# Gjerman/Orange3-Spark

Hardware: AMD Instinct MI355X
Metric: samples/sec LogisticRegression.fit on 1Bx256 synthetic at 1/2/4/8 MI355X (higher is better)
Workload: dtype bf16; 1 GPU; global_batch=1000000000, seq_len=256, features=256, parallelism=dp1, resident_rows=497795896, lineage_rows=502204104, device=cuda:0

## Files before the change

### orange3_spark_amd/ops/csrc/glm.hip

```cpp
#include <type_traits>

#include "common.h"

using namespace o3s;

namespace {

enum { LOSS_LOGISTIC = 0, LOSS_HINGE = 1, LOSS_SQUARED = 2 };

constexpr int kBlock = 256;
constexpr int kWavesPerBlock = kBlock / kWave;

__host__ __device__ __forceinline__ uint32_t umad24(uint32_t a, uint32_t c, uint32_t add) {
#if defined(__HIP_DEVICE_COMPILE__)
  return __umul24(a, c) + add;
#else
  return (a & 0xFFFFFFu) * c + add;
#endif
}
__host__ __device__ __forceinline__ uint32_t mix24(uint32_t h) {
  h ^= h >> 16;
  h = umad24(h, 0xED5AD4u, h);
  h ^= h >> 15;
  return umad24(h, 0x2C1B3Cu, h);
// ... 268 lines not shown
  wtshift *= kSynthShift;
  float acc_r = 0.f, acc_loss = 0.f, acc_w = 0.f;

  const int64_t ntiles = (n + RT - 1) / RT;
  const int64_t gw = (int64_t)blockIdx.x * kWavesPerBlock + wid;
  const int64_t nw = (int64_t)gridDim.x * kWavesPerBlock;
  for (int64_t t = gw; t < ntiles; t += nw) {
    const int64_t base = t * RT;
    short8 xv[UNROLL][CPL];
    float xf[UNROLL][CPL][8];
#pragma unroll
    for (int u = 0; u < UNROLL; ++u) {
      const int64_t row = base + u * G + g;
      const bool ok = row < n;
      const int64_t rowc = ok ? row : n - 1;
      const uint32_t rk = SRC == 1 ? feat_key(seed, row0 + row) : 0u;
#pragma unroll
      for (int k = 0; k < CPL; ++k) {
        const int ch = c + k * LPR;
        if (SRC == 0) {
          const bool okc = ok && ch < nch;
          const int chc = ch < nch ? ch : nch - 1;
          short8 v = __builtin_nontemporal_load(reinterpret_cast<const short8*>(X + rowc * ld + 8 * chc));
          xv[u][k] = okc ? v : short8{0, 0, 0, 0, 0, 0, 0, 0};
        } else {
          const uint32_t h0 = synth_word(rk, 2 * ch), h1 = synth_word(rk, 2 * ch + 1);
#pragma unroll
          for (int j = 0; j < 4; ++j) {
            xf[u][k][j] = synth_byte(h0, j);
            xf[u][k][4 + j] = synth_byte(h1, j);
          }
        }
      }
    }
    float yy[NF], ww[NF];
#pragma unroll
    for (int j = 0; j < NF; ++j) {
      const int64_t row = base + (ubase + j) * G + g;
      const bool ok = row < n;
      const int64_t rowc = ok ? row : n - 1;
      if (SRC == 0) {
        const float yv = y[rowc];
        const float wv = sw ? sw[rowc] : 1.f;
        yy[j] = ok ? yv : 0.f;
        ww[j] = ok ? wv : 0.f;
      } else {
        ww[j] = ok ? 1.f : 0.f;
      }
    }
    float dot[UNROLL], dtrue[UNROLL];
#pragma unroll
    for (int u = 0; u < UNROLL; ++u) {
      float d = SRC == 1 ? wshift : 0.f, dt = wtshift;
#pragma unroll
      for (int k = 0; k < CPL; ++k) {
        float x[8];
        if (SRC == 0) {
          unpack8(xv[u][k], x);
        } else {
#pragma unroll
          for (int j = 0; j < 8; ++j) x[j] = xf[u][k][j];
        }
#pragma unroll
        for (int j = 0; j < 8; ++j) {
          d = fmaf(x[j], w[k][j], d);
          if (SRC == 1) dt = fmaf(x[j], wt[k][j], dt);
        }
      }
      dot[u] = d;
      dtrue[u] = dt;
    }
    RR::run(dot, c);
    if (SRC == 1) {
      RR::run(dtrue, c);
#pragma unroll
      for (int j = 0; j < NF; ++j) {
        const int64_t row = base + (ubase + j) * G + g;
        yy[j] = synth_label(row_key(seed, row0 + row), dtrue[j] + btrue);
      }
    }
    float res[NF];
#pragma unroll
    for (int j = 0; j < NF; ++j) {
      float r, l;
      loss_terms<LOSS>(dot[j] + intercept, yy[j], ww[j], r, l);
      res[j] = r;
      if (rep) { acc_r += r; acc_loss += l; acc_w += ww[j]; }
    }
#pragma unroll
    for (int u = 0; u < UNROLL; ++u)
#pragma unroll
      for (int k = 0; k < CPL; ++k) {
        if (SRC == 0) asm volatile("" : "+v"(xv[u][k]));
        else {
#pragma unroll
          for (int j = 0; j < 8; ++j) asm volatile("" : "+v"(xf[u][k][j]));
        }
      }
#pragma unroll
    for (int u = 0; u < UNROLL; ++u) {
      float r = __shfl(res[u % NF], g * LPR + RR::owner(u), kWave);
      if (SRC == 1) { rs += r; r *= kSynthScale; }
#pragma unroll
      for (int k = 0; k < CPL; ++k) {
        float x[8];
        if (SRC == 0) {
          unpack8(xv[u][k], x);
        } else {
#pragma unroll
          for (int j = 0; j < 8; ++j) x[j] = xf[u][k][j];
        }
#pragma unroll
        for (int j = 0; j < 8; ++j) acc[k][j] = fmaf(r, x[j], acc[k][j]);
      }
    }
  }

  if (SRC == 1) {
#pragma unroll
    for (int k = 0; k < CPL; ++k)
#pragma unroll
      for (int j = 0; j < 8; ++j) acc[k][j] = fmaf(rs, kSynthShift, acc[k][j]);
  }
  grad_epilogue<LPR, CPL>(acc, acc_r, acc_loss, acc_w, partial, pstride, 0, lane, wid, c);
}


template <int CTRL>
__device__ __forceinline__ float dpp_f(float v) {
  return __builtin_bit_cast(float, __builtin_amdgcn_update_dpp(0, __builtin_bit_cast(int, v), CTRL, 0xF, 0xF,
                                                               false));
}
constexpr int kDppXor1 = 0xB1, kDppXor2 = 0x4E, kDppHalfMirror = 0x141;
__device__ __forceinline__ void row_reduce_8x2(float (&v)[2], int c) {
  v[0] += dpp_f<kDppXor1>(v[0]);
  v[1] += dpp_f<kDppXor1>(v[1]);
  v[0] += dpp_f<kDppXor2>(v[0]);
  v[1] += dpp_f<kDppXor2>(v[1]);
  const bool up = (c & 4) != 0;
  const float keep = up ? v[1] : v[0], send = up ? v[0] : v[1];
  v[0] = keep + dpp_f<kDppHalfMirror>(send);
}

struct RowSampler {
  uint32_t key, thr;
  int64_t grow0;
  __device__ __forceinline__ bool on() const { return thr < (1u << 24); }
  __device__ __forceinline__ bool keep(int64_t row) const { return (row_key(key, grow0 + row) >> 8) < thr; }
};
__host__ __device__ __forceinline__ uint32_t sample_key(uint32_t seed, uint32_t iter) {
  return fmix32(seed ^ fmix32(iter * 0x9E3779B1u + 0x7F4A7C15u));
}

constexpr int kStgTileBytes = 8 * 1024, kStgLabelBytes = kWave * 4;
constexpr int kStgWaveBytes = kStgTileBytes + 2 * kStgLabelBytes;
constexpr int kStgLd = 256;
constexpr unsigned kAuxNt = 2;
struct TileStage {
  static constexpr int LPR = 8, CPL = 4, UNROLL = 2, G = kWave / LPR, kTileOps = 1 + UNROLL * CPL;
  unsigned char* slot;
  uint32_t sbase;
  const unsigned char* xs;
  const float* yrs;
  const float* yls;
  int64_t tstep;
  uint32_t r_ahead, l_ahead;
  bool lab_younger;

  __device__ static __forceinline__ uint32_t fresh(int v) {
    asm volatile("" : "+v"(v));
    return (uint32_t)v;
  }
  __device__ static __forceinline__ uint32_t label_off(uint32_t g, uint32_t c) { return ((c >> 2) * G + g) * 4; }

  __device__ __forceinline__ void issue_tile(int g, int c) {
    const uint32_t gg = fresh(g), cc = fresh(c);
    __builtin_amdgcn_global_load_lds(reinterpret_cast<const unsigned char*>(yrs) + label_off(gg, cc),
                                     slot + kStgTileBytes, 4, 0, 0);
    const uint32_t xoff = gg * (kStgLd * 2) + cc * 16;
#pragma unroll
    for (int u = 0; u < UNROLL; ++u)
#pragma unroll
      for (int k = 0; k < CPL; ++k)
        __builtin_amdgcn_global_load_lds(xs + (u * G * kStgLd * 2 + k * LPR * 16) + xoff, slot + (u * CPL + k) * 1024,
                                         16, 0, kAuxNt);
    xs += tstep * (kStgLd * 2);
    yrs += tstep;
    --r_ahead;
    lab_younger = false;
  }
  __device__ __forceinline__ void issue_label(int g, int c) {
    __builtin_amdgcn_global_load_lds(reinterpret_cast<const unsigned char*>(yls) + label_off(fresh(g), fresh(c)),
                                     slot + kStgTileBytes + kStgLabelBytes, 4, 0, 0);
    yls += tstep;
    --l_ahead;
    lab_younger = true;
  }
  __device__ __forceinline__ void take_tile(int g, int c, short8 (&xv)[UNROLL][CPL], float& yv) {
    if (lab_younger) asm volatile("s_waitcnt vmcnt(1)" ::: "memory");
    else asm volatile("s_waitcnt vmcnt(0)" ::: "memory");
    const uint32_t lane = fresh(g) * LPR + fresh(c);
    asm volatile(
        "ds_read_b128 %0, %9\n\t"
        "ds_read_b128 %1, %9 offset:1024\n\t"
        "ds_read_b128 %2, %9 offset:2048\n\t"
        "ds_read_b128 %3, %9 offset:3072\n\t"
        "ds_read_b128 %4, %9 offset:4096\n\t"
        "ds_read_b128 %5, %9 offset:5120\n\t"
        "ds_read_b128 %6, %9 offset:6144\n\t"
        "ds_read_b128 %7, %9 offset:7168\n\t"
        "ds_read_b32 %8, %10 offset:8192\n\t"
        "s_waitcnt lgkmcnt(0)"
        : "=&v"(xv[0][0]), "=&v"(xv[0][1]), "=&v"(xv[0][2]), "=&v"(xv[0][3]), "=&v"(xv[1][0]), "=&v"(xv[1][1]),
          "=&v"(xv[1][2]), "=&v"(xv[1][3]), "=&v"(yv)
        : "v"(sbase + lane * 16), "v"(sbase + lane * 4)
        : "memory");
    if (r_ahead > 0) issue_tile(g, c);
    __builtin_amdgcn_sched_barrier(0);
  }
  __device__ __forceinline__ void take_label(int g, int c, float& yv) {
    if (lab_younger) asm volatile("s_waitcnt vmcnt(0)" ::: "memory");
    else asm volatile("s_waitcnt vmcnt(%0)" ::"n"(kTileOps) : "memory");
    const uint32_t a4 = sbase + (fresh(g) * LPR + fresh(c)) * 4;
    asm volatile("ds_read_b32 %0, %1 offset:8448\n\ts_waitcnt lgkmcnt(0)" : "=v"(yv) : "v"(a4) : "memory");
    lab_younger = false;
    if (l_ahead > 0) issue_label(g, c);
  }
};
static_assert(kStgTileBytes == 8192 && kStgLabelBytes == 256, "the asm offsets in TileStage");

template <class SRC, int LPR, int CPL, int UNROLL, int LOSS, bool SMP, bool FULL = false, bool STAGED = false>
__device__ __forceinline__ void grad_tile(
    int64_t base, int64_t n, const typename SRC::elem* __restrict__ X, int64_t ld, int nch,
    const float* __restrict__ y, const float* __restrict__ sw, uint32_t seed, int64_t row0, const float (&w)[CPL][8],
    float wshift, float intercept, int g, int c, const RowSampler smp, float (&acc)[CPL][8], float& rs, float& acc_r,
    float& acc_loss, float& acc_w, TileStage* stg = nullptr) {
  constexpr int G = kWave / LPR;
  using RR = RowReduce<LPR, UNROLL>;
  constexpr int NF = RR::NF;
  static_assert(!STAGED || (FULL && NF == 1 && LPR == TileStage::LPR && CPL == TileStage::CPL && UNROLL == TileStage::UNROLL),
                "the staged slot holds one (8, 4, 2) tile");
  const int ubase = RR::base(c);
  const bool rep = RR::representative(c);
  typename SRC::chunk xv[UNROLL][CPL];
#pragma unroll
  for (int u = 0; u < UNROLL; ++u) {
    const int64_t row = base + u * G + g;
    const bool ok = row < n;
    const int64_t rowc = ok ? row : n - 1;
    const uint32_t fk = SRC::kLineage ? feat_key(seed, row0 + row) : 0u;
#pragma unroll
    for (int k = 0; k < CPL; ++k) {
      const int ch = c + k * LPR;
      if constexpr (SRC::kLineage) {
        SRC::decode(synth_word(fk, 2 * ch), synth_word(fk, 2 * ch + 1), xv[u][k]);
      } else if constexpr (STAGED) {
      } else if constexpr (FULL) {
        SRC::load(X, ld, row, ch, xv[u][k]);
      } else {
        const int chc = ch < nch ? ch : nch - 1;
        SRC::load(X, ld, rowc, chc, xv[u][k]);
        SRC::mask(xv[u][k], ok && ch < nch);
      }
    }
  }
  float yy[NF], ww[NF];
#pragma unroll
  for (int j = 0; j < NF; ++j) {
    const int64_t row = base + (ubase + j) * G + g;
    const bool ok = row < n;
    const int64_t rowc = ok ? row : n - 1;
    if constexpr (STAGED) {
      if constexpr (!SRC::kLineage) stg->take_tile(g, c, xv, yy[j]);
      ww[j] = 1.f;
    } else if constexpr (FULL) {
      yy[j] = y[row];
      ww[j] = sw ? sw[row] : 1.f;
    } else {
      const float yv = y[rowc];
      const float wv = sw ? sw[rowc] : 1.f;
      yy[j] = ok ? yv : 0.f;
      ww[j] = ok ? wv : 0.f;
    }
    if constexpr (SMP && !STAGED) {
      if (!smp.keep(row)) ww[j] = 0.f;
    }
  }
  float dot[UNROLL];
#pragma unroll
  for (int u = 0; u < UNROLL; ++u) {
    float2_ d2 = {0.f, 0.f};
#pragma unroll
    for (int k = 0; k < CPL; ++k) {
      float x[8];
      SRC::unpack(xv[u][k], x);
#pragma unroll
      for (int j = 0; j < 8; j += 2) {
        const float2_ xx = {x[j], x[j + 1]}, ww2 = {w[k][j], w[k][j + 1]};
        d2 = __builtin_elementwise_fma(xx, ww2, d2);
      }
    }
    dot[u] = SRC::dot(d2.x + d2.y, wshift);
  }
  constexpr bool kDpp = LPR == 8 && UNROLL == 2;
  if constexpr (kDpp) row_reduce_8x2(dot, c);
  else RR::run(dot, c);
  if constexpr (STAGED && SRC::kLineage) stg->take_label(g, c, yy[0]);
  if constexpr (STAGED && SMP) {
    if (!smp.keep(base + (int64_t)TileStage::fresh(ubase * G + g))) ww[0] = 0.f;
  }
  float res[NF];
#pragma unroll
  for (int j = 0; j < NF; ++j) {
    float r, l;
    loss_terms<LOSS>(dot[j] + intercept, yy[j], ww[j], r, l);
    res[j] = r;
    if (rep) { acc_r += r; acc_loss += l; acc_w += ww[j]; }
  }
#pragma unroll
  for (int u = 0; u < UNROLL; ++u)
#pragma unroll
    for (int k = 0; k < CPL; ++k) SRC::pin(xv[u][k]);
  float other = 0.f;
  if constexpr (kDpp) other = dpp_f<kDppHalfMirror>(res[0]);
#pragma unroll
  for (int u = 0; u < UNROLL; ++u) {
    float r;
    if constexpr (kDpp) r = ((c & 4) != 0) == (u == 0) ? other : res[0];
    else r = __shfl(res[u % NF], g * LPR + RR::owner(u), kWave);
    r = SRC::resid(r, rs);
#pragma unroll
    for (int k = 0; k < CPL; ++k) {
      float x[8];
      SRC::unpack(xv[u][k], x);
#pragma unroll
      for (int j = 0; j < 8; ++j) acc[k][j] = fmaf(r, x[j], acc[k][j]);
    }
  }
}

template <int LPR, int CPL, int UNROLL, int LOSS, int MW, bool SMP, bool FULL = false>
__global__ __launch_bounds__(kBlock, MW) void glm_grad_mixed_kernel(
    const uint16_t* __restrict__ X, int64_t ld, int64_t n_res, const float* __restrict__ y,
    const float* __restrict__ sw, const float* __restrict__ y_lin, const float* __restrict__ sw_lin,
    const float* __restrict__ coef, const float* __restrict__ bptr, uint32_t seed, int64_t row0, int64_t n_lin,
    float* __restrict__ partial, int pstride, int64_t res_row0, const int64_t* __restrict__ t_dev, uint32_t sseed,
    uint32_t sthr, int pacc) {
  constexpr int G = kWave / LPR;
  constexpr int RT = G * UNROLL;
  const int lane = threadIdx.x & (kWave - 1);
  const int wid = threadIdx.x / kWave;
  const int g = lane / LPR, c = lane % LPR;
  const int nch = (int)(ld / 8);
  const float intercept = *bptr;
  const uint32_t skey = SMP ? sample_key(sseed, (uint32_t)((t_dev ? t_dev[0] : 0) + 1)) : 0u;
  const RowSampler smp_res{skey, sthr, res_row0}, smp_lin{skey, sthr, row0};

  float w[CPL][8], acc[CPL][8];
  float wshift = 0.f;
#pragma unroll
  for (int k = 0; k < CPL; ++k)
#pragma unroll
    for (int j = 0; j < 8; ++j) {
      const int col = 8 * (c + k * LPR) + j;
      w[k][j] = col < ld ? coef[col] : 0.f;
      wshift += w[k][j];
      acc[k][j] = 0.f;
    }
  wshift *= kSynthShift;
  float rs = 0.f;
  float acc_r = 0.f, acc_loss = 0.f, acc_w = 0.f;

  const int64_t Tr = (n_res + RT - 1) / RT, Tl = (n_lin + RT - 1) / RT, S = Tr + Tl;
  const int64_t gw = (int64_t)blockIdx.x * kWavesPerBlock + wid;
  const int64_t nw = (int64_t)gridDim.x * kWavesPerBlock;
  if (gw < S) {
    int64_t L = gw * Tl / S, rem = gw * Tl - L * S;
    const int64_t q0 = nw * Tl / S, r0 = nw * Tl - q0 * S;
    for (int64_t s = gw; s < S; s += nw) {
      if (rem + Tl >= S)
        grad_tile<RowsLineage, LPR, CPL, UNROLL, LOSS, SMP, FULL>(L * RT, n_lin, X, ld, nch, y_lin, sw_lin, seed, row0, w,
                                                                  wshift, intercept, g, c, smp_lin, acc, rs, acc_r, acc_loss,
                                                                  acc_w);
      else
        grad_tile<RowsBf16, LPR, CPL, UNROLL, LOSS, SMP, FULL>((s - L) * RT, n_res, X, ld, nch, y, sw, seed, row0, w, wshift,
                                                               intercept, g, c, smp_res, acc, rs, acc_r, acc_loss, acc_w);
      rem += r0;
      L += q0;
      if (rem >= S) { rem -= S; ++L; }
    }
  }
#pragma unroll
  for (int k = 0; k < CPL; ++k)
#pragma unroll
    for (int j = 0; j < 8; ++j) acc[k][j] = fmaf(rs, kSynthShift, acc[k][j]);
  grad_epilogue<LPR, CPL>(acc, acc_r, acc_loss, acc_w, partial, pstride, pacc, lane, wid, c);
}

template <int LOSS, bool SMP>
__global__ __launch_bounds__(kBlock, 3) void glm_grad_staged_kernel(
    const uint16_t* __restrict__ X, int64_t n_res, const float* __restrict__ y, const float* __restrict__ y_lin,
    const float* __restrict__ coef, const float* __restrict__ bptr, uint32_t seed, int64_t row0, int64_t n_lin,
    float* __restrict__ partial, int pstride, int64_t res_row0, const int64_t* __restrict__ t_dev, uint32_t sseed,
    uint32_t sthr, int pacc) {
  constexpr int LPR = TileStage::LPR, CPL = TileStage::CPL, UNROLL = TileStage::UNROLL, G = TileStage::G;
  constexpr int RT = G * UNROLL;
  constexpr int64_t ld = kStgLd;
  __shared__ __attribute__((aligned(16))) unsigned char slots[kWavesPerBlock * kStgWaveBytes];
  const int lane = threadIdx.x & (kWave - 1);
  const int wid = __builtin_amdgcn_readfirstlane(threadIdx.x / kWave);
  const int g = lane / LPR, c = lane % LPR;
  const float intercept = *bptr;
  const uint32_t skey = SMP ? sample_key(sseed, (uint32_t)((t_dev ? t_dev[0] : 0) + 1)) : 0u;
  const RowSampler smp_res{skey, sthr, res_row0}, smp_lin{skey, sthr, row0};

  float w[CPL][8], acc[CPL][8];
  float wshift = 0.f;
#pragma unroll
  for (int k = 0; k < CPL; ++k)
#pragma unroll
    for (int j = 0; j < 8; ++j) {
      w[k][j] = coef[8 * (c + k * LPR) + j];
      wshift += w[k][j];
      acc[k][j] = 0.f;
    }
  wshift *= kSynthShift;
  float rs = 0.f;
  float acc_r = 0.f, acc_loss = 0.f, acc_w = 0.f;

  const uint32_t Tr = (uint32_t)(n_res / RT), Tl = (uint32_t)(n_lin / RT);
  const uint32_t gw = blockIdx.x * kWavesPerBlock + wid, nw = gridDim.x * kWavesPerBlock;
  const uint32_t nr = gw < Tr ? (Tr - gw + nw - 1) / nw : 0u;
  const uint32_t nl = gw < Tl ? (Tl - gw + nw - 1) / nw : 0u;
  const uint32_t S = nr + nl;
  int64_t br = (int64_t)gw * RT, bl = br;
  using lds_byte = __attribute__((address_space(3))) unsigned char;
  TileStage st{slots + wid * kStgWaveBytes,
               (uint32_t)(uintptr_t)(lds_byte*)slots + wid * kStgWaveBytes,
               reinterpret_cast<const unsigned char*>(X + br * ld),
               y + br,
               y_lin + bl,
               (int64_t)nw * RT,
               nr,
               nl,
               false};
  static_assert(RowReduce<LPR, UNROLL>::NF == 1, "TileStage::label_off: one label per lane");
  if (nl > 0) st.issue_label(g, c);
  if (nr > 0) st.issue_tile(g, c);
  uint32_t rem = 0;
  for (uint32_t s = 0; s < S; ++s) {
    rem += nl;
    if (rem >= S) {
      rem -= S;
      grad_tile<RowsLineage, LPR, CPL, UNROLL, LOSS, SMP, true, true>(bl, n_lin, X, ld, CPL * LPR, y_lin, nullptr, seed, row0,
                                                                      w, wshift, intercept, g, c, smp_lin, acc, rs, acc_r,
                                                                      acc_loss, acc_w, &st);
      bl += st.tstep;
    } else {
      grad_tile<RowsBf16, LPR, CPL, UNROLL, LOSS, SMP, true, true>(br, n_res, X, ld, CPL * LPR, y, nullptr, seed, row0, w,
                                                                   wshift, intercept, g, c, smp_res, acc, rs, acc_r,
                                                                   acc_loss, acc_w, &st);
      br += st.tstep;
    }
  }
#pragma unroll
  for (int k = 0; k < CPL; ++k)
#pragma unroll
    for (int j = 0; j < 8; ++j) acc[k][j] = fmaf(rs, kSynthShift, acc[k][j]);
  grad_epilogue<LPR, CPL>(acc, acc_r, acc_loss, acc_w, partial, pstride, pacc, lane, wid, c);
}

template <class SRC, int LPR, int CPL, int U, bool UNW, bool FULL = false>
__device__ __forceinline__ void stats_tile(int64_t base, int64_t n, const typename SRC::elem* __restrict__ X,
                                           int64_t ld, int nch, const float* __restrict__ y,
                                           const float* __restrict__ sw, uint32_t seed, int64_t row0, int g, int c,
                                           float2_ (&s1)[CPL][4], float2_ (&s2)[CPL][4], float2_ (&syx)[CPL][4],
                                           float (&rsum)[3]) {
  constexpr int G = kWave / LPR;
  typename SRC::chunk xv[U][CPL];
  uint32_t fk[U];
  float yv[U], wv[U];
#pragma unroll
  for (int u = 0; u < U; ++u) {
    const int64_t row = base + u * G + g;
    const bool ok = row < n;
    const int64_t rowc = FULL ? row : (ok ? row : n - 1);
    yv[u] = y[rowc];
    if (UNW) {
      wv[u] = 1.f;
    } else if constexpr (FULL) {
      wv[u] = sw[row];
    } else {
      const float w0 = sw ? sw[rowc] : 1.f;
      wv[u] = ok ? w0 : 0.f;
    }
    if constexpr (SRC::kLineage) {
      fk[u] = feat_key(seed, row0 + rowc);
    } else {
#pragma unroll
      for (int k = 0; k < CPL; ++k) {
        const int ch = c + k * LPR;
        if constexpr (FULL) {
          SRC::load(X, ld, row, ch, xv[u][k]);
        } else {
          SRC::load(X, ld, rowc, ch < nch ? ch : nch - 1, xv[u][k]);
          SRC::mask(xv[u][k], ch < nch);
        }
      }
    }
  }
#pragma unroll
  for (int u = 0; u < U; ++u) {
    const float2_ w2 = {wv[u], wv[u]};
    const float wy = wv[u] * yv[u];
    const float2_ wy2 = {wy, wy};
#pragma unroll
    for (int k = 0; k < CPL; ++k) {
      float x[8];
      if constexpr (SRC::kLineage) {
        SRC::load(fk[u], c + k * LPR, xv[u][k]);
        SRC::values(xv[u][k], x);
      } else {
        SRC::unpack(xv[u][k], x);
      }
#pragma unroll
      for (int j = 0; j < 4; ++j) {
        const float2_ xx = {x[2 * j], x[2 * j + 1]};
        const float2_ wx = UNW ? xx : w2 * xx;
        s1[k][j] += wx;
        s2[k][j] = __builtin_elementwise_fma(wx, xx, s2[k][j]);
        syx[k][j] = __builtin_elementwise_fma(wy2, xx, syx[k][j]);
      }
    }
    if (c == 0) {
      rsum[0] += wv[u];
      rsum[1] += wy;
      rsum[2] = fmaf(wy, yv[u], rsum[2]);
    }
  }
}
template <int LPR, int CPL>
__device__ __forceinline__ void stats_epilogue(const float2_ (&s1)[CPL][4], const float2_ (&s2)[CPL][4],
                                               const float2_ (&syx)[CPL][4], const float (&rsum)[3],
                                               float* __restrict__ partial, int pstride, int lane, int wid, int c) {
  constexpr int DP = LPR * CPL * 8;
  __shared__ float red[kWavesPerBlock][3 * DP + 4];
#pragma unroll
  for (int k = 0; k < CPL; ++k)
#pragma unroll
    for (int j = 0; j < 4; ++j)
#pragma unroll
      for (int h = 0; h < 2; ++h) {
        float a = s1[k][j][h], b = s2[k][j][h], e = syx[k][j][h];
#pragma unroll
        for (int off = LPR; off < kWave; off <<= 1) {
          a += __shfl_xor(a, off, kWave);
          b += __shfl_xor(b, off, kWave);
          e += __shfl_xor(e, off, kWave);
        }
        const int col = 8 * (c + k * LPR) + 2 * j + h;
        if (lane < LPR) {
          red[wid][col] = a;
          red[wid][DP + col] = b;
          red[wid][2 * DP + col] = e;
        }
      }
#pragma unroll
  for (int q = 0; q < 3; ++q) {
    const float v = wave_sum(rsum[q]);
    if (lane == 0) red[wid][3 * DP + q] = v;
  }
  __syncthreads();
  for (int i = threadIdx.x; i < 3 * DP + 3; i += kBlock) {
    float s = 0.f;
#pragma unroll
    for (int q = 0; q < kWavesPerBlock; ++q) s += red[q][i];
    partial[(int64_t)blockIdx.x * pstride + i] = s;
  }
}

template <int LPR, int CPL, int MW, int FULL = 0>
__global__ __launch_bounds__(kBlock, MW) void glm_stats_mixed_kernel(
    const uint16_t* __restrict__ X, int64_t ld, int64_t n_res, const float* __restrict__ y,
    const float* __restrict__ sw, const float* __restrict__ y_lin, const float* __restrict__ sw_lin, uint32_t seed,
    int64_t row0, int64_t n_lin, float* __restrict__ partial, int pstride) {
  constexpr int G = kWave / LPR;
  constexpr int U = CPL >= 8 ? 1 : 8 / CPL;
  constexpr int RT = G * U;
  const int lane = threadIdx.x & (kWave - 1);
  const int wid = threadIdx.x / kWave;
  const int g = lane / LPR, c = lane % LPR;
  const int nch = (int)(ld / 8);
  float2_ s1[CPL][4], s2[CPL][4], syx[CPL][4];
#pragma unroll
  for (int k = 0; k < CPL; ++k)
#pragma unroll
    for (int j = 0; j < 4; ++j) s1[k][j] = s2[k][j] = syx[k][j] = float2_{0.f, 0.f};
  float rsum[3] = {0.f, 0.f, 0.f};
  const int64_t Tr = (n_res + RT - 1) / RT, Tl = (n_lin + RT - 1) / RT, S = Tr + Tl;
  const int64_t gw = (int64_t)blockIdx.x * kWavesPerBlock + wid;
  const int64_t nw = (int64_t)gridDim.x * kWavesPerBlock;
  if (gw < S) {
    int64_t L = gw * Tl / S, rem = gw * Tl - L * S;
    const int64_t q0 = nw * Tl / S, r0 = nw * Tl - q0 * S;
    for (int64_t s = gw; s < S; s += nw) {
      if constexpr (FULL != 0) {
        if (rem + Tl >= S)
          stats_tile<RowsLineage, LPR, CPL, U, FULL == 1, true>(L * RT, n_lin, X, ld, nch, y_lin, sw_lin, seed, row0, g, c,
                                                               s1, s2, syx, rsum);
        else
          stats_tile<RowsBf16, LPR, CPL, U, FULL == 1, true>((s - L) * RT, n_res, X, ld, nch, y, sw, seed, row0, g, c, s1,
                                                            s2, syx, rsum);
      } else if (rem + Tl >= S) {
        const int64_t base = L * RT;
// ... 845 lines not shown
    if constexpr (kDpp) row_reduce_8x2(dot, c);
    else RR::run(dot, c);
    float res[NF];
#pragma unroll
    for (int j = 0; j < NF; ++j) {
      float r, l;
      loss_terms<LOSS>(dot[j] + intercept, yy[j], ww[j], r, l);
      res[j] = r;
      if (rep) { acc_r += r; acc_loss += l; acc_w += ww[j]; }
    }
    float other = 0.f;
    if constexpr (kDpp) other = dpp_f<kDppHalfMirror>(res[0]);
#pragma unroll
    for (int u = 0; u < UNROLL; ++u) {
      float r;
      if constexpr (kDpp) r = ((c & 4) != 0) == (u == 0) ? other : res[0];
      else r = __shfl(res[u % NF], g * LPR + RR::owner(u), kWave);
#pragma unroll
      for (int k = 0; k < CPL; ++k)
#pragma unroll
        for (int h = 0; h < 2; ++h)
#pragma unroll
          for (int j = 0; j < 4; ++j) acc[k][4 * h + j] = fmaf(r, xv[u][k][h][j], acc[k][4 * h + j]);
    }
  }

  grad_epilogue<LPR, CPL>(acc, acc_r, acc_loss, acc_w, partial, pstride, pacc, lane, wid, c);
}

template <int LPR, int CPL, int U, int MW>
__global__ __launch_bounds__(kBlock, MW) void glm_stats_f32_kernel(
    const float* __restrict__ X, int64_t ld, int64_t n, const float* __restrict__ y, const float* __restrict__ sw,
    float* __restrict__ partial, int pstride) {
  constexpr int RT = kWave / LPR * U;
  const int lane = threadIdx.x & (kWave - 1);
  const int wid = threadIdx.x / kWave;
  const int g = lane / LPR, c = lane % LPR;
  const int nch = (int)(ld / 8);
  float2_ s1[CPL][4], s2[CPL][4], syx[CPL][4];
#pragma unroll
  for (int k = 0; k < CPL; ++k)
#pragma unroll
    for (int j = 0; j < 4; ++j) s1[k][j] = s2[k][j] = syx[k][j] = float2_{0.f, 0.f};
  float rsum[3] = {0.f, 0.f, 0.f};
  const int64_t ntiles = (n + RT - 1) / RT;
  const int64_t gw = (int64_t)blockIdx.x * kWavesPerBlock + wid;
  const int64_t nw = (int64_t)gridDim.x * kWavesPerBlock;
  for (int64_t t = gw; t < ntiles; t += nw) {
    const int64_t base = t * RT;
    if (sw == nullptr && base + RT <= n)
      stats_tile<RowsF32, LPR, CPL, U, true>(base, n, X, ld, nch, y, sw, 0u, 0, g, c, s1, s2, syx, rsum);
    else
      stats_tile<RowsF32, LPR, CPL, U, false>(base, n, X, ld, nch, y, sw, 0u, 0, g, c, s1, s2, syx, rsum);
  }
  stats_epilogue<LPR, CPL>(s1, s2, syx, rsum, partial, pstride, lane, wid, c);
}

template <int LPR, int CPL>
__global__ __launch_bounds__(kBlock) void glm_margin_f32_kernel(
    const float* __restrict__ X, int64_t ld, int64_t n, const float* __restrict__ coef, float intercept,
    float* __restrict__ out) {
  margin_body<RowsF32, LPR, CPL, (CPL >= 4 ? 1 : 4 / CPL)>(X, ld, n, coef, intercept, out);
}

template <int LPR, int CPL>
__global__ __launch_bounds__(kBlock) void glm_colstats_f32_kernel(
    const float* __restrict__ X, int64_t ld, int64_t n, const float* __restrict__ sw, float* __restrict__ partial,
    int pstride) {
  colstats_body<RowsF32, LPR, CPL>(X, ld, n, sw, 0u, 0, partial, pstride);
}

template <int C> struct F32Cfg { static constexpr int U = C >= 8 ? 1 : 8 / C, MW = C >= 8 ? 1 : 2; };

}

O3S_API int o3s_glm_grad_f32(int loss, const void* X, int64_t ld, int64_t n, const float* y, const float* sw,
                             const float* coef, int64_t n_lin, float* partial, int grid, double* out,
                             int accumulate, int64_t res_row0, const int64_t* t_dev, uint32_t sseed, uint32_t sthr,
                             int splits, hipStream_t st) {
  Layout l;
  if (ld <= 0 || !resolve_layout(ld, &l) || grid <= 0 || n < 0 || n_lin != 0) return -1;
  const int pstride = l.dpad + 4;
  const float* Xf = (const float*)X;
  const bool smp = sthr < (1u << 24);
  const int rc = for_row_slices(splits, n, 0, [&](int64_t r_lo, int64_t r_n, int64_t, int64_t, int pacc) {
    return with_remapped_layout_and_loss(l, loss, [&](auto L, auto C, auto LOSS) {
      constexpr int U = F32Cfg<C>::U, MW = F32Cfg<C>::MW;
      auto go = [&](auto SMP) {
        launch(glm_grad_f32_kernel<L, C, U, LOSS, MW, SMP>, grid, st, Xf + r_lo * ld, ld, r_n, y + r_lo,
               sw ? sw + r_lo : nullptr, coef, coef + l.dpad, partial, pstride, res_row0 + r_lo, t_dev, sseed, sthr,
               pacc);
      };
      if (smp) go(std::true_type{});
      else go(std::false_type{});
      return 0;
    });
  });
  if (rc != 0) return rc;
  return launch_finish(partial, grid, pstride, l.dpad + 3, out, accumulate, st);
}

O3S_API int o3s_glm_stats_f32(const void* X, int64_t ld, int64_t n, const float* y, const float* sw, int64_t n_lin,
                              float* partial, int grid, double* out, hipStream_t st) {
  Layout l;
  if (ld <= 0 || !resolve_layout(ld, &l) || grid <= 0 || n < 0 || n_lin != 0) return -1;
  const int pstride = 3 * l.dpad + 4;
  const int rc = with_remapped_layout(l, [&](auto L, auto C) {
    if constexpr (C > 4) {
      return -2;
    } else {
      launch(glm_stats_f32_kernel<L, C, (C >= 4 ? 1 : 4 / C), 2>, grid, st, (const float*)X, ld, n, y, sw, partial,
             pstride);
      return 0;
    }
  });
  if (rc != 0) return rc;
  return launch_finish(partial, grid, pstride, 3 * l.dpad + 3, out, 0, st);
}

O3S_API int o3s_glm_margin_f32(const void* X, int64_t ld, int64_t n, const float* coef, float intercept, float* out,
                               int grid, hipStream_t st) {
  Layout l;
  if (ld <= 0 || !resolve_layout(ld, &l) || grid <= 0) return -1;
  if (n <= 0) return 0;
  return with_remapped_layout(l, [&](auto L, auto C) {
    launch(glm_margin_f32_kernel<L, C>, grid, st, (const float*)X, ld, n, coef,
           intercept, out);
    O3S_CHECK_LAUNCH();
    return 0;
  });
}

O3S_API int o3s_glm_colstats_f32(const void* X, int64_t ld, int64_t n, const float* sw, float* partial, int grid,
                                 double* out, hipStream_t st) {
  Layout l;
  if (ld <= 0 || !resolve_layout(ld, &l) || grid <= 0 || n < 0) return -1;
  const int pstride = 2 * l.dpad + 2;
  if (n > 0) {
    const int rc = with_remapped_layout(l, [&](auto L, auto C) {
      launch(glm_colstats_f32_kernel<L, C>, grid, st, (const float*)X, ld, n, sw,
             partial, pstride);
      return 0;
    });
    if (rc != 0) return rc;
  } else {
    hipMemsetAsync(partial, 0, sizeof(float) * pstride * (size_t)grid, st);
  }
  return launch_finish(partial, grid, pstride, 2 * l.dpad + 1, out, 0, st);
}

namespace {

typedef uint32_t sm_u32x4 __attribute__((ext_vector_type(4)));
typedef __bf16 sm_bf16x2 __attribute__((ext_vector_type(2)));

__device__ __forceinline__ uint32_t pk_bf16(float a, float b) {
  float2_ v;
  v[0] = a;
  v[1] = b;
  return __builtin_bit_cast(uint32_t, __builtin_convertvector(v, sm_bf16x2));
}

__device__ __forceinline__ void split8(const float4_ a, const float4_ b, sm_bf16x8& hi, sm_bf16x8& mid,
                                       sm_bf16x8& lo) {
  sm_u32x4 ph, pm, pl;
#pragma unroll
  for (int j = 0; j < 4; ++j) {
    const float x0 = j < 2 ? a[2 * j] : b[2 * j - 4], x1 = j < 2 ? a[2 * j + 1] : b[2 * j - 3];
    ph[j] = pk_bf16(x0, x1);
    const float r0 = x0 - __uint_as_float(ph[j] << 16), r1 = x1 - __uint_as_float(ph[j] & 0xffff0000u);
    pm[j] = pk_bf16(r0, r1);
    pl[j] = pk_bf16(r0 - __uint_as_float(pm[j] << 16), r1 - __uint_as_float(pm[j] & 0xffff0000u));
  }
  hi = __builtin_bit_cast(sm_bf16x8, ph);
  mid = __builtin_bit_cast(sm_bf16x8, pm);
  lo = __builtin_bit_cast(sm_bf16x8, pl);
}

template <int NB>
__global__ __launch_bounds__(kSmThreads, 1) void glm_softmax_f32_kernel(
    const float* __restrict__ X, int64_t n, int64_t ldx, const int32_t* __restrict__ y,
    const float* __restrict__ sw, const uint16_t* __restrict__ Wsp, const float* __restrict__ bias, int K,
    float* __restrict__ partial, int pstride) {
  using L = SmLds<NB>;
  constexpr int D = L::D, KS = 2 * NB, WLD = L::WLD, XLD = L::XLD, RLD = L::RLD;
  __shared__ __attribute__((aligned(16))) uint16_t smem[L::ELEMS];
  __shared__ __attribute__((aligned(16))) float bs[32];
  const int lane = threadIdx.x & 63, wid = threadIdx.x >> 6;
  const int r = lane & 31, h = lane >> 5;
  uint16_t* Ws = smem;
  uint16_t* Xs = smem + L::W_ELEMS + wid * L::WAVE_ELEMS;
  uint16_t* Rs = Xs + 32 * XLD;

  for (int p = threadIdx.x; p < 3 * 32 * (D / 8); p += kSmThreads) {
    const int row = p / (D / 8), k8 = p % (D / 8);
    *reinterpret_cast<sm_bf16x8*>(Ws + row * WLD + k8 * 8) =
        *reinterpret_cast<const sm_bf16x8*>(Wsp + (int64_t)row * D + k8 * 8);
  }
  auto cv = [](int v) { return 8 * (v >> 2) + (v & 3); };
  if (threadIdx.x < 32) bs[threadIdx.x] = (int)threadIdx.x < K ? bias[threadIdx.x] : -INFINITY;
  uint16_t* Rw = Rs + 4 * h * RLD + r;
  __syncthreads();

  sm_f32x16 G[NB];
#pragma unroll
  for (int b = 0; b < NB; ++b)
#pragma unroll
    for (int v = 0; v < 16; ++v) G[b][v] = 0.f;
  float gb[16];
#pragma unroll
  for (int v = 0; v < 16; ++v) gb[v] = 0.f;
  float lossacc = 0.f;

  const int64_t ntiles = (n + 31) / 32;
  const int64_t step = (int64_t)gridDim.x * kSmWaves;
  int64_t tile = (int64_t)blockIdx.x * kSmWaves + wid;
  float4_ xf[KS][2], xn[KS][2];
  auto load = [&](int64_t t, float4_ (*dst)[2]) {
    int64_t row = t * 32 + r;
    row = row < n ? row : n - 1;
    const float* src = X + row * ldx;
#pragma unroll
    for (int ks = 0; ks < KS; ++ks) {
      const int col = ks * 16 + 8 * h;
      if (col < ldx) {
        dst[ks][0] = *reinterpret_cast<const float4_*>(src + col);
        dst[ks][1] = *reinterpret_cast<const float4_*>(src + col + 4);
      } else {
#pragma unroll
        for (int j = 0; j < 4; ++j) dst[ks][0][j] = dst[ks][1][j] = 0.f;
      }
    }
  };
  if (tile < ntiles) load(tile, xf);
  for (; tile < ntiles; tile += step) {
    if (tile + step < ntiles) load(tile + step, xn);
    const int64_t row = tile * 32 + r;
    const bool valid = row < n;
    const int ylh = (valid ? y[row] : -1) - 4 * h;
    const float wr = valid ? (sw ? sw[row] : 1.f) : 0.f;
    sm_f32x16 acc;
#pragma unroll
    for (int j = 0; j < 4; ++j) {
      const float4_ b4 = *reinterpret_cast<const float4_*>(bs + 8 * j + 4 * h);
#pragma unroll
      for (int u = 0; u < 4; ++u) acc[4 * j + u] = b4[u];
    }
    sm_bf16x8 xh[KS], xm[KS];
#pragma unroll
    for (int ks = 0; ks < KS; ++ks) {
      sm_bf16x8 xl;
      split8(xf[ks][0], xf[ks][1], xh[ks], xm[ks], xl);
      const uint16_t* wp = Ws + r * WLD + ks * 16 + 8 * h;
      const sm_bf16x8 a0 = *reinterpret_cast<const sm_bf16x8*>(wp);
      const sm_bf16x8 a1 = *reinterpret_cast<const sm_bf16x8*>(wp + 32 * WLD);
      const sm_bf16x8 a2 = *reinterpret_cast<const sm_bf16x8*>(wp + 64 * WLD);
      acc = __builtin_amdgcn_mfma_f32_32x32x16_bf16(a0, xl, acc, 0, 0, 0);
      acc = __builtin_amdgcn_mfma_f32_32x32x16_bf16(a2, xh[ks], acc, 0, 0, 0);
      acc = __builtin_amdgcn_mfma_f32_32x32x16_bf16(a1, xm[ks], acc, 0, 0, 0);
      acc = __builtin_amdgcn_mfma_f32_32x32x16_bf16(a0, xm[ks], acc, 0, 0, 0);
      acc = __builtin_amdgcn_mfma_f32_32x32x16_bf16(a1, xh[ks], acc, 0, 0, 0);
      acc = __builtin_amdgcn_mfma_f32_32x32x16_bf16(a0, xh[ks], acc, 0, 0, 0);
      __builtin_amdgcn_sched_barrier(0);
    }
    float mx = -INFINITY;
#pragma unroll
    for (int v = 0; v < 16; ++v) mx = fmaxf(mx, acc[v]);
    mx = fmaxf(mx, __shfl_xor(mx, 32, 64));
    float se = 0.f;
#pragma unroll
    for (int v = 0; v < 16; ++v) se += __expf(acc[v] - mx);
    se += __shfl_xor(se, 32, 64);
    const float lse = mx + __logf(se);
#pragma unroll
    for (int v = 0; v < 16; v += 2) {
      float rv[2];
#pragma unroll
      for (int u = 0; u < 2; ++u) {
        const bool hit = cv(v + u) == ylh;
        rv[u] = wr * (__expf(acc[v + u] - lse) - (hit ? 1.f : 0.f));
        gb[v + u] += rv[u];
        if (hit) lossacc += wr * (lse - acc[v + u]);
      }
      const uint32_t ph = pk_bf16(rv[0], rv[1]);
      const uint32_t pl = pk_bf16(rv[0] - __uint_as_float(ph << 16), rv[1] - __uint_as_float(ph & 0xffff0000u));
      Rw[cv(v) * RLD] = (uint16_t)ph;
      Rw[cv(v + 1) * RLD] = (uint16_t)(ph >> 16);
      Rw[(32 + cv(v)) * RLD] = (uint16_t)pl;
      Rw[(32 + cv(v + 1)) * RLD] = (uint16_t)(pl >> 16);
    }
    asm volatile("s_waitcnt lgkmcnt(0)" ::: "memory");
    __builtin_amdgcn_wave_barrier();
    sm_bf16x8 ar[2][2];
#pragma unroll
    for (int rs = 0; rs < 2; ++rs)
#pragma unroll
      for (int s = 0; s < 2; ++s)
        ar[rs][s] = *reinterpret_cast<const sm_bf16x8*>(Rs + (s * 32 + r) * RLD + rs * 16 + 8 * h);
#pragma unroll
    for (int rs = 0; rs < 2; ++rs) {
      if ((r >> 4) == rs) {
#pragma unroll
        for (int ks = 0; ks < KS; ++ks) {
          *reinterpret_cast<sm_bf16x8*>(Xs + (r & 15) * XLD + ks * 16 + 8 * h) = xh[ks];
          *reinterpret_cast<sm_bf16x8*>(Xs + (16 + (r & 15)) * XLD + ks * 16 + 8 * h) = xm[ks];
        }
      }
      asm volatile("s_waitcnt lgkmcnt(0)" ::: "memory");
      __builtin_amdgcn_wave_barrier();
#pragma unroll
      for (int b = 0; b < NB; ++b) {
        sm_bf16x8 bh, bm;
#pragma unroll
        for (int q = 0; q < 8; ++q) {
// ... 65 lines not shown
```

Before: 23.47 billion samples/s.

## Compute staged resident-row margins with bf16 MFMA against a three-way split weight

```diff
diff --git a/orange3_spark_amd/ops/csrc/glm.hip b/orange3_spark_amd/ops/csrc/glm.hip
--- a/orange3_spark_amd/ops/csrc/glm.hip
+++ b/orange3_spark_amd/ops/csrc/glm.hip
@@ -444,14 +444,24 @@
   return fmix32(seed ^ fmix32(iter * 0x9E3779B1u + 0x7F4A7C15u));
 }
 
+typedef __bf16 sm_bf16x2 __attribute__((ext_vector_type(2)));
+__device__ __forceinline__ uint32_t pk_bf16(float a, float b) {
+  float2_ v;
+  v[0] = a;
+  v[1] = b;
+  return __builtin_bit_cast(uint32_t, __builtin_convertvector(v, sm_bf16x2));
+}
+
 constexpr int kStgTileBytes = 8 * 1024, kStgLabelBytes = kWave * 4;
 constexpr int kStgWaveBytes = kStgTileBytes + 2 * kStgLabelBytes;
+constexpr int kStgFragBytes = 8 * 1024;
 constexpr int kStgLd = 256;
 constexpr unsigned kAuxNt = 2;
 struct TileStage {
   static constexpr int LPR = 8, CPL = 4, UNROLL = 2, G = kWave / LPR, kTileOps = 1 + UNROLL * CPL;
   unsigned char* slot;
   uint32_t sbase;
+  uint32_t fbase;
   const unsigned char* xs;
   const float* yrs;
   const float* yls;
@@ -465,11 +475,11 @@
   }
   __device__ static __forceinline__ uint32_t label_off(uint32_t g, uint32_t c) { return ((c >> 2) * G + g) * 4; }
 
-  __device__ __forceinline__ void issue_tile(int g, int c) {
-    const uint32_t gg = fresh(g), cc = fresh(c);
-    __builtin_amdgcn_global_load_lds(reinterpret_cast<const unsigned char*>(yrs) + label_off(gg, cc),
+  __device__ __forceinline__ void issue_tile(int lane) {
+    const uint32_t ln = fresh(lane);
+    __builtin_amdgcn_global_load_lds(reinterpret_cast<const unsigned char*>(yrs) + (ln & 15) * 4,
                                      slot + kStgTileBytes, 4, 0, 0);
-    const uint32_t xoff = gg * (kStgLd * 2) + cc * 16;
+    const uint32_t xoff = (ln >> 3) * (kStgLd * 2) + ((ln ^ (ln >> 4)) & 7) * 16;
 #pragma unroll
     for (int u = 0; u < UNROLL; ++u)
 #pragma unroll
@@ -488,27 +498,78 @@
     --l_ahead;
     lab_younger = true;
   }
-  __device__ __forceinline__ void take_tile(int g, int c, short8 (&xv)[UNROLL][CPL], float& yv) {
+  __device__ __forceinline__ void take_tile(int lane, short8 (&xb)[8], short8 (&xv)[UNROLL][CPL], float& yv,
+                                            short8 (&fa)[3]) {
     if (lab_younger) asm volatile("s_waitcnt vmcnt(1)" ::: "memory");
     else asm volatile("s_waitcnt vmcnt(0)" ::: "memory");
-    const uint32_t lane = fresh(g) * LPR + fresh(c);
+    const uint32_t ln = fresh(lane);
+    const uint32_t b0 = sbase + ((ln & 8) << 9) + ((ln >> 4) << 10) + ((ln & 7) << 7) + (((ln >> 1) & 3) << 4);
     asm volatile(
-        "ds_read_b128 %0, %9\n\t"
-        "ds_read_b128 %1, %9 offset:1024\n\t"
-        "ds_read_b128 %2, %9 offset:2048\n\t"
-        "ds_read_b128 %3, %9 offset:3072\n\t"
-        "ds_read_b128 %4, %9 offset:4096\n\t"
-        "ds_read_b128 %5, %9 offset:5120\n\t"
-        "ds_read_b128 %6, %9 offset:6144\n\t"
-        "ds_read_b128 %7, %9 offset:7168\n\t"
-        "ds_read_b32 %8, %10 offset:8192\n\t"
+        "ds_read_b128 %17, %26\n\t"
+        "ds_read_b128 %18, %26 offset:1024\n\t"
+        "ds_read_b128 %19, %26 offset:2048\n\t"
+        "ds_read_b128 %0, %20\n\t"
+        "ds_read_b128 %1, %21\n\t"
+        "ds_read_b128 %2, %22\n\t"
+        "ds_read_b128 %3, %23\n\t"
+        "ds_read_b128 %4, %20 offset:64\n\t"
+        "ds_read_b128 %5, %21 offset:64\n\t"
+        "ds_read_b128 %6, %22 offset:64\n\t"
+        "ds_read_b128 %7, %23 offset:64\n\t"
+        "ds_read_b128 %8, %24\n\t"
+        "ds_read_b128 %9, %24 offset:1024\n\t"
+        "ds_read_b128 %10, %24 offset:2048\n\t"
+        "ds_read_b128 %11, %24 offset:3072\n\t"
+        "ds_read_b128 %12, %24 offset:4096\n\t"
+        "ds_read_b128 %13, %24 offset:5120\n\t"
+        "ds_read_b128 %14, %24 offset:6144\n\t"
+        "ds_read_b128 %15, %24 offset:7168\n\t"
+        "ds_read_b32 %16, %25 offset:8192\n\t"
         "s_waitcnt lgkmcnt(0)"
-        : "=&v"(xv[0][0]), "=&v"(xv[0][1]), "=&v"(xv[0][2]), "=&v"(xv[0][3]), "=&v"(xv[1][0]), "=&v"(xv[1][1]),
-          "=&v"(xv[1][2]), "=&v"(xv[1][3]), "=&v"(yv)
-        : "v"(sbase + lane * 16), "v"(sbase + lane * 4)
+        : "=&v"(xb[0]), "=&v"(xb[1]), "=&v"(xb[2]), "=&v"(xb[3]), "=&v"(xb[4]), "=&v"(xb[5]), "=&v"(xb[6]),
+          "=&v"(xb[7]), "=&v"(xv[0][0]), "=&v"(xv[0][1]), "=&v"(xv[0][2]), "=&v"(xv[0][3]), "=&v"(xv[1][0]),
+          "=&v"(xv[1][1]), "=&v"(xv[1][2]), "=&v"(xv[1][3]), "=&v"(yv), "=&v"(fa[0]), "=&v"(fa[1]), "=&v"(fa[2])
+        : "v"(b0), "v"(b0 ^ 16u), "v"(b0 ^ 32u), "v"(b0 ^ 48u), "v"(sbase + ((ln ^ (ln >> 4)) << 4)),
+          "v"(sbase + ln * 4), "v"(fbase + ln * 16)
         : "memory");
-    if (r_ahead > 0) issue_tile(g, c);
+    if (r_ahead > 0) issue_tile(lane);
     __builtin_amdgcn_sched_barrier(0);
+  }
+  __device__ __forceinline__ float4_ dot(int lane, const short8 (&xb)[8], short8 (&fa)[3]) {
+    float4_ d;
+    asm volatile(
+        "v_mfma_f32_16x16x32_bf16 %0, %1, %5, 0\n\t"
+        "s_nop 7\n\t"
+        "ds_read_b128 %1, %4 offset:3072\n\t"
+        "v_mfma_f32_16x16x32_bf16 %0, %2, %6, %0\n\t"
+        "s_nop 7\n\t"
+        "ds_read_b128 %2, %4 offset:4096\n\t"
+        "v_mfma_f32_16x16x32_bf16 %0, %3, %7, %0\n\t"
+        "s_nop 7\n\t"
+        "ds_read_b128 %3, %4 offset:5120\n\t"
+        "s_waitcnt lgkmcnt(2)\n\t"
+        "v_mfma_f32_16x16x32_bf16 %0, %1, %8, %0\n\t"
+        "s_nop 7\n\t"
+        "ds_read_b128 %1, %4 offset:6144\n\t"
+        "s_waitcnt lgkmcnt(2)\n\t"
+        "v_mfma_f32_16x16x32_bf16 %0, %2, %9, %0\n\t"
+        "s_nop 7\n\t"
+        "ds_read_b128 %2, %4 offset:7168\n\t"
+        "s_waitcnt lgkmcnt(2)\n\t"
+        "v_mfma_f32_16x16x32_bf16 %0, %3, %10, %0\n\t"
+        "s_nop 7\n\t"
+        "s_waitcnt lgkmcnt(1)\n\t"
+        "v_mfma_f32_16x16x32_bf16 %0, %1, %11, %0\n\t"
+        "s_nop 7\n\t"
+        "s_waitcnt lgkmcnt(0)\n\t"
+        "v_mfma_f32_16x16x32_bf16 %0, %2, %12, %0\n\t"
+        "s_nop 7\n\t"
+        "s_nop 3"
+        : "=&v"(d), "+v"(fa[0]), "+v"(fa[1]), "+v"(fa[2])
+        : "v"(fbase + fresh(lane) * 16), "v"(xb[0]), "v"(xb[1]), "v"(xb[2]), "v"(xb[3]), "v"(xb[4]), "v"(xb[5]),
+          "v"(xb[6]), "v"(xb[7])
+        : "memory");
+    return d;
   }
   __device__ __forceinline__ void take_label(int g, int c, float& yv) {
     if (lab_younger) asm volatile("s_waitcnt vmcnt(0)" ::: "memory");
@@ -530,14 +591,15 @@
   constexpr int G = kWave / LPR;
   using RR = RowReduce<LPR, UNROLL>;
   constexpr int NF = RR::NF;
-  static_assert(!STAGED || (FULL && NF == 1 && LPR == TileStage::LPR && CPL == TileStage::CPL && UNROLL == TileStage::UNROLL),
-                "the staged slot holds one (8, 4, 2) tile");
+  static_assert(!STAGED || (SRC::kLineage && FULL && NF == 1 && LPR == TileStage::LPR && CPL == TileStage::CPL &&
+                            UNROLL == TileStage::UNROLL),
+                "the staged slot holds the labels of one (8, 4, 2) lineage tile");
   const int ubase = RR::base(c);
   const bool rep = RR::representative(c);
   typename SRC::chunk xv[UNROLL][CPL];
 #pragma unroll
   for (int u = 0; u < UNROLL; ++u) {
-    const int64_t row = base + u * G + g;
+    const int64_t row = base + u * G + (STAGED ? (int)TileStage::fresh(g) : g);
     const bool ok = row < n;
     const int64_t rowc = ok ? row : n - 1;
     const uint32_t fk = SRC::kLineage ? feat_key(seed, row0 + row) : 0u;
@@ -546,7 +608,6 @@
       const int ch = c + k * LPR;
       if constexpr (SRC::kLineage) {
         SRC::decode(synth_word(fk, 2 * ch), synth_word(fk, 2 * ch + 1), xv[u][k]);
-      } else if constexpr (STAGED) {
       } else if constexpr (FULL) {
         SRC::load(X, ld, row, ch, xv[u][k]);
       } else {
@@ -563,7 +624,6 @@
     const bool ok = row < n;
     const int64_t rowc = ok ? row : n - 1;
     if constexpr (STAGED) {
-      if constexpr (!SRC::kLineage) stg->take_tile(g, c, xv, yy[j]);
       ww[j] = 1.f;
     } else if constexpr (FULL) {
       yy[j] = y[row];
@@ -629,6 +689,42 @@
       for (int j = 0; j < 8; ++j) acc[k][j] = fmaf(r, x[j], acc[k][j]);
     }
   }
+}
+
+template <int LOSS, bool SMP>
+__device__ __forceinline__ void staged_resident_tile(int64_t base, float intercept, int lane, const RowSampler smp,
+                                                     float (&acc)[TileStage::CPL][8], float& acc_r, float& acc_loss,
+                                                     float& acc_w, TileStage* stg) {
+  constexpr int CPL = TileStage::CPL, UNROLL = TileStage::UNROLL;
+  short8 xb[8], xv[UNROLL][CPL];
+  float yv;
+  short8 fa[3];
+  stg->take_tile(lane, xb, xv, yv, fa);
+  const float4_ d = stg->dot(lane, xb, fa);
+  float wv = 1.f;
+  if constexpr (SMP) {
+    if (!smp.keep(base + (int64_t)(TileStage::fresh(lane) & 15u))) wv = 0.f;
+  }
+  float r, l;
+  loss_terms<LOSS>(((d[2] + d[1]) + d[0]) + intercept, yv, wv, r, l);
+  if (lane < 16) { acc_r += r; acc_loss += l; acc_w += wv; }
+#pragma unroll
+  for (int u = 0; u < UNROLL; ++u)
+#pragma unroll
+    for (int k = 0; k < CPL; ++k) RowsBf16::pin(xv[u][k]);
+  const int src = (int)(TileStage::fresh(lane) >> 3) * 4;
+  const float rr[UNROLL] = {
+      __builtin_bit_cast(float, __builtin_amdgcn_ds_bpermute(src, __builtin_bit_cast(int, r))),
+      __builtin_bit_cast(float, __builtin_amdgcn_ds_bpermute(src + 32, __builtin_bit_cast(int, r)))};
+#pragma unroll
+  for (int u = 0; u < UNROLL; ++u)
+#pragma unroll
+    for (int k = 0; k < CPL; ++k) {
+      float x[8];
+      unpack8(xv[u][k], x);
+#pragma unroll
+      for (int j = 0; j < 8; ++j) acc[k][j] = fmaf(rr[u], x[j], acc[k][j]);
+    }
 }
 
 template <int LPR, int CPL, int UNROLL, int LOSS, int MW, bool SMP, bool FULL = false>
@@ -698,7 +794,9 @@
   constexpr int LPR = TileStage::LPR, CPL = TileStage::CPL, UNROLL = TileStage::UNROLL, G = TileStage::G;
   constexpr int RT = G * UNROLL;
   constexpr int64_t ld = kStgLd;
-  __shared__ __attribute__((aligned(16))) unsigned char slots[kWavesPerBlock * kStgWaveBytes];
+  __shared__ __attribute__((aligned(256))) unsigned char slots[kWavesPerBlock * kStgWaveBytes];
+  __shared__ __attribute__((aligned(256))) unsigned char frags[kStgFragBytes];
+  static_assert(kStgWaveBytes % 256 == 0, "TileStage: a slot starts on a bank row");
   const int lane = threadIdx.x & (kWave - 1);
   const int wid = __builtin_amdgcn_readfirstlane(threadIdx.x / kWave);
   const int g = lane / LPR, c = lane % LPR;
@@ -727,8 +825,29 @@
   const uint32_t S = nr + nl;
   int64_t br = (int64_t)gw * RT, bl = br;
   using lds_byte = __attribute__((address_space(3))) unsigned char;
+  for (int e = threadIdx.x; e < kStgFragBytes / 16; e += kBlock) {
+    const int s = e >> 6, term = e & 15, q = (e & 63) >> 4;
+    uint32_t p[4] = {0u, 0u, 0u, 0u};
+    if (term < 3) {
+      const float* cw = coef + 8 * (8 * q + s);
+#pragma unroll
+      for (int j = 0; j < 4; ++j) {
+        const float x0 = cw[2 * j], x1 = cw[2 * j + 1];
+        const uint32_t ph = pk_bf16(x0, x1);
+        const float r0 = x0 - __uint_as_float(ph << 16), r1 = x1 - __uint_as_float(ph & 0xffff0000u);
+        const uint32_t pm = pk_bf16(r0, r1);
+        const uint32_t pl = pk_bf16(r0 - __uint_as_float(pm << 16), r1 - __uint_as_float(pm & 0xffff0000u));
+        p[j] = term == 0 ? ph : term == 1 ? pm : pl;
+      }
+    }
+    uint32_t* const dst = reinterpret_cast<uint32_t*>(frags + e * 16);
+#pragma unroll
+    for (int j = 0; j < 4; ++j) dst[j] = p[j];
+  }
+  __syncthreads();
   TileStage st{slots + wid * kStgWaveBytes,
                (uint32_t)(uintptr_t)(lds_byte*)slots + wid * kStgWaveBytes,
+               (uint32_t)(uintptr_t)(lds_byte*)frags,
                reinterpret_cast<const unsigned char*>(X + br * ld),
                y + br,
                y_lin + bl,
@@ -738,7 +857,7 @@
                false};
   static_assert(RowReduce<LPR, UNROLL>::NF == 1, "TileStage::label_off: one label per lane");
   if (nl > 0) st.issue_label(g, c);
-  if (nr > 0) st.issue_tile(g, c);
+  if (nr > 0) st.issue_tile(lane);
   uint32_t rem = 0;
   for (uint32_t s = 0; s < S; ++s) {
     rem += nl;
@@ -749,9 +868,7 @@
                                                                       acc_loss, acc_w, &st);
       bl += st.tstep;
     } else {
-      grad_tile<RowsBf16, LPR, CPL, UNROLL, LOSS, SMP, true, true>(br, n_res, X, ld, CPL * LPR, y, nullptr, seed, row0, w,
-                                                                   wshift, intercept, g, c, smp_res, acc, rs, acc_r,
-                                                                   acc_loss, acc_w, &st);
+      staged_resident_tile<LOSS, SMP>(br, intercept, lane, smp_res, acc, acc_r, acc_loss, acc_w, &st);
       br += st.tstep;
     }
   }
@@ -1903,14 +2020,6 @@
 namespace {
 
 typedef uint32_t sm_u32x4 __attribute__((ext_vector_type(4)));
-typedef __bf16 sm_bf16x2 __attribute__((ext_vector_type(2)));
-
-__device__ __forceinline__ uint32_t pk_bf16(float a, float b) {
-  float2_ v;
-  v[0] = a;
-  v[1] = b;
-  return __builtin_bit_cast(uint32_t, __builtin_convertvector(v, sm_bf16x2));
-}
 
 __device__ __forceinline__ void split8(const float4_ a, const float4_ b, sm_bf16x8& hi, sm_bf16x8& mid,
                                        sm_bf16x8& lo) {
```

Result: faster. 24.01 billion samples/s (median of 6 runs) (+2.3%).
